# MahdiGhafoorian/NLML_HPE

Measured on AMD Instinct MI355X. Metric: faces_per_sec, higher is better.
Workload: dtype f16x2s

## Files before the change

nlml_hpe_amd/csrc/encoder_heads_f16x2_w8.hip:

```cpp
#include <hip/hip_runtime.h>

#include "../../include/nlml_hpe.h"
#include "abi_internal.h"
#include "ipd_norm.h"
#include "encoder_heads_f16x2_dev.h"
#include "layout.h"

namespace nlml {
namespace hx {

template <typename XHi, typename XLo, typename Extra>
__device__ __forceinline__ void step_w8(f32x16 (&acc)[2][2], f32x16 (&accS)[2][2], const h8 (&wcur)[2][2], const h8 (&xh)[2], h8 (&xl)[2],
                                        h8 (&wnext_hi)[2][2], const h8* __restrict__ wp_hi, h8 (&wnext_lo)[2][2], const h8* __restrict__ wp_lo,
                                        XHi xload_hi, XLo xload_lo, Extra extra) {
#pragma unroll
  for (int m = 0; m < 12; ++m) {
    const int t = m / 4, nb = (m % 4) / 2, fb = m % 2;
    if (t == 0) accS[nb][fb] = __builtin_amdgcn_mfma_f32_32x32x16_f16(wcur[nb][1], xh[fb], accS[nb][fb], 0, 0, 0);
    else if (t == 1) accS[nb][fb] = __builtin_amdgcn_mfma_f32_32x32x16_f16(wcur[nb][0], xl[fb], accS[nb][fb], 0, 0, 0);
    else acc[nb][fb] = __builtin_amdgcn_mfma_f32_32x32x16_f16(wcur[nb][0], xh[fb], acc[nb][fb], 0, 0, 0);
    __builtin_amdgcn_sched_barrier(0);
    if (m == 0) xload_hi(0);
    if (m == 1) xload_hi(1);
    if (m == 2) wnext_hi[0][0] = wp_hi[0];
    if (m == 4) wnext_lo[0][1] = wp_lo[64];
    if (m == 6) wnext_hi[1][0] = wp_hi[128];
    if (m == 8) xload_lo(0);
    if (m == 9) xload_lo(1);
    if (m == 10) wnext_lo[1][1] = wp_lo[192];
    extra(m);
    __builtin_amdgcn_sched_barrier(0);
  }
}

template <bool VEC4, bool NORM>
__device__ __forceinline__ void stage_e0_pass_w8(const Ctx& c, const Args& a, int64_t row0, int tid, int pass, int jw, int nbh,
                                                 f32x16 (&acc)[2][2], f32x16 (&accS)[2][2]) {
  constexpr int NB = 2, NFB = 2;
  constexpr int WSTEP = 4 * 2 * 64;
  const int F = a.F;
  const int nslab = (int)c.hdr.k8_e0 / XS_STEPS;

  const int srow = tid >> 3, scol = (tid & 7) * 4;
  int64_t r = row0 + srow;
  const bool live = r < a.B;
  r = live ? r : a.B - 1;
  const float* p = a.x + r * a.ldx;
  double ipd = 1.0, rcp = 1.0, ra = 0.0, rb = 0.0, rc = 0.0;
  if (NORM) {
    double x0, y0, z0;
    ipd_setup(p, ipd, rcp, x0, y0, z0);
    ipd_phase(scol % 3, x0, y0, z0, ra, rb, rc);
  }
  unsigned nzbits = 0u;

  struct Set { float v[4]; };
  auto gload = [&](int s, Set& st) {
    s = s < nslab ? s : nslab - 1;
    const int k = s * XS_COLS + scol;
    if (VEC4) {
      const int kc = k < F ? k : (NORM ? k - 12 * ((k - F + 15) / 12) : F - 4);
      const f32x4 t = *reinterpret_cast<const f32x4*>(p + kc);
#pragma unroll
      for (int e = 0; e < 4; ++e) st.v[e] = t[e];
    } else {
#pragma unroll
      for (int e = 0; e < 4; ++e) st.v[e] = p[k + e < F ? k + e : F - 1];
    }
  };
  auto lw_begin = [&](Set& st) {
#pragma unroll
    for (int e = 0; e < 4; ++e) asm volatile("" : "+v"(st.v[e]));
  };
  auto lw_norm = [&](Set& st, int q) {
    const int t = q % 3;
    const double rr = t == 0 ? ra : (t == 1 ? rb : rc);
    st.v[q] = (float)div_ipd((double)st.v[q] - rr, ipd, rcp);
  };
  auto lw_rotate = [&]() {
    const double t0 = rc; rc = rb; rb = ra; ra = t0;
  };
  typedef unsigned u2 __attribute__((ext_vector_type(2)));
  unsigned pend_hi[2], pend_lo[2];
  auto lw_split = [&](Set& st, int j, bool real_slab) {
    const unsigned m = real_slab ? 0x7fffffffu : 0u;
    nzbits |= (__float_as_uint(st.v[2 * j]) | __float_as_uint(st.v[2 * j + 1])) & m;
    split2(st.v[2 * j], st.v[2 * j + 1], pend_hi[j], pend_lo[j]);
  };
  constexpr int XW_PLANE = 64 * 64, XW_SLAB = 2 * XW_PLANE, XW_BUF = 2 * XW_SLAB, O_XW = LDS_BYTES - 2 * XW_BUF;
  static_assert(O_XW >= 16 * 512 * 16, "slabs behind the parked accumulators");
  const int wr_off = srow * 64 + ((((tid & 7) >> 1) ^ ((srow >> 2) & 3)) << 4) + 8 * (tid & 1);
  auto lw_store = [&](int slab_off, int piece) {
    char* d = c.lds + O_XW + slab_off + wr_off;
    if (piece == 0) *reinterpret_cast<u2*>(d) = u2{pend_hi[0], pend_hi[1]};
    else *reinterpret_cast<u2*>(d + XW_PLANE) = u2{pend_lo[0], pend_lo[1]};
  };
  auto lwrite = [&](int slab_off, Set& st, bool real_slab) {
    lw_begin(st);
    if (NORM) {
#pragma unroll
      for (int q = 0; q < 4; ++q) lw_norm(st, q);
      lw_rotate();
    }
#pragma unroll
    for (int j = 0; j < 2; ++j) lw_split(st, j, real_slab);
    lw_store(slab_off, 0);
    lw_store(slab_off, 1);
  };

  const int job = 4 * pass + jw;
  load_bias<NB, NFB>(acc, c.blob4 + c.hdr.b_off(ST_E0) + job * (4 * 8) + (2 * nbh) * 8, c.h);
  zero_acc<NB, NFB>(accS);
  const h8* w = c.blob8 + c.hdr.w_off(ST_E0) + (size_t)job * c.hdr.job_w16(ST_E0) + (2 * nbh * 2) * 64 + c.lane;
  auto wfrag = [&](int ks) { return w + (size_t)ks * WSTEP; };

  Set set[2];
#ifndef W8_D0_HI
#define W8_D0_HI 2
#endif
#ifndef W8_D0_LO
#define W8_D0_LO 2
#endif
  constexpr int R0 = 4, DH = W8_D0_HI, DL = W8_D0_LO;
  h8 wr[R0][NB][2];
  gload(0, set[0]);
  gload(1, set[1]);
  lwrite(0, set[0], true);
  lwrite(XW_SLAB, set[1], true);
  gload(2, set[0]);
  gload(3, set[1]);
#pragma unroll
  for (int d = 0; d < (DH > DL ? DH : DL); ++d)
#pragma unroll
    for (int nb = 0; nb < NB; ++nb)
#pragma unroll
      for (int pp = 0; pp < 2; ++pp)
        if (d < (pp ? DL : DH)) wr[d][nb][pp] = wfrag(d)[(nb * 2 + pp) * 64];
  __syncthreads();

  const int rd0 = c.f * 64 + ((c.h ^ ((c.f >> 2) & 3)) << 4);
  typedef __attribute__((address_space(3))) const char LdsC;
  LdsC* const xb0 = (LdsC*)(c.lds + O_XW + rd0);
  LdsC* const xb1 = (LdsC*)(c.lds + O_XW + (rd0 ^ 32));
  h8 xh[2][NFB], xl[NFB];
  auto xread = [&](LdsC* base, int t, int fb, int pp) {
    return *reinterpret_cast<const __attribute__((address_space(3))) h8*>(base + (t >> 1) * XW_SLAB + pp * XW_PLANE + fb * (32 * 64));
  };
  const int niter = nslab / 2;
#pragma unroll
  for (int fb = 0; fb < NFB; ++fb) {
    xh[0][fb] = xread(xb0, 0, fb, 0);
    xl[fb] = xread(xb0, 0, fb, 1);
  }
  int cur = 0, nxt = XW_BUF;
  for (int it = 0; it < niter; ++it) {
    const int s = 2 * it;
    LdsC* xc[2] = {xb0 + cur, xb1 + cur};
    LdsC* xn = xb0 + nxt;
    asm volatile("" : "+v"(xc[0]), "+v"(xc[1]), "+v"(xn));
#pragma unroll
    for (int t = 0; t < 4; ++t) {
      const int ks = 4 * it + t;
      if (t == 3) __syncthreads();
      step_w8(acc, accS, wr[t], xh[t & 1], xl, wr[(t + DH) % R0], wfrag(ks + DH), wr[(t + DL) % R0], wfrag(ks + DL),
              [&](int fb) { xh[(t + 1) & 1][fb] = t < 3 ? xread(xc[(t + 1) & 1], t + 1, fb, 0) : xread(xn, 0, fb, 0); },
              [&](int fb) { xl[fb] = t < 3 ? xread(xc[(t + 1) & 1], t + 1, fb, 1) : xread(xn, 0, fb, 1); },
              [&](int m) {
                if (t >= 2) return;
                Set& st = set[t & 1];
                const int j = m;
                const bool real = s + t + 2 < nslab;
                if (j == 0) lw_begin(st);
                if (NORM && j >= 1 && j < 5) lw_norm(st, j - 1);
                if (NORM && j == 5) lw_rotate();
                if (j == 6 || j == 7) lw_split(st, j - 6, real);
                if (j == 8) lw_store(nxt + t * XW_SLAB, 0);
                if (j == 9) lw_store(nxt + t * XW_SLAB, 1);
                if (j == 11) gload(s + t + 4, st);
              });
    }
    const int t0 = cur; cur = nxt; nxt = t0;
  }
  if (pass == 0 && a.valid) {
    const unsigned long long m = __ballot(nzbits != 0u);
    if ((tid & 7) == 0 && live) a.valid[row0 + srow] = ((m >> (c.lane & 56)) & 0xFFull) ? 1 : 0;
  }
}

#ifdef HX_STAMPS
#define W8S(i)                                                                                                          \
  do {                                                                                                                  \
    if (a.latent && c.lane == 0)                                                                                        \
      reinterpret_cast<unsigned long long*>(a.latent)[((size_t)blockIdx.x * 8 + c.wv) * 16 + (i)] = __builtin_amdgcn_s_memtime(); \
  } while (0)
#define W8S_WALL(i)                                                                                                     \
  do {                                                                                                                  \
    if (a.latent && c.lane == 0)                                                                                        \
      reinterpret_cast<unsigned long long*>(a.latent)[((size_t)blockIdx.x * 8 + c.wv) * 16 + (i)] = wall_clock64();     \
  } while (0)
#else
#define W8S(i) do { } while (0)
#define W8S_WALL(i) do { } while (0)
#endif

template <bool VEC4, bool NORM, bool TRUNK = false>
__global__ __launch_bounds__(512) void encoder_heads_f16x2_w8_kernel(Args a) {
  __shared__ __attribute__((aligned(16))) char lds[LDS_BYTES];

  const int tid = threadIdx.x;
  Ctx c;
  c.blob8 = reinterpret_cast<const h8*>(a.blob);
  c.blob4 = reinterpret_cast<const f32x4*>(a.blob);
  c.hdr = load_hdr(reinterpret_cast<const Header*>(a.blob));
  c.lds = lds;
  c.lane = tid & 63;
  c.f = c.lane & 31;
  c.h = c.lane >> 5;
  c.wv = __builtin_amdgcn_readfirstlane(tid >> 6);
  const int jw = c.wv >> 1, nbh = c.wv & 1;
  const int64_t row0 = (int64_t)blockIdx.x * TILE_FACES;

  {
    constexpr int WSTEP1 = 4 * 2 * 64;
    const h8* w1 = c.blob8 + c.hdr.w_off(ST_E1) + (size_t)jw * c.hdr.job_w16(ST_E1) + (2 * nbh * 2) * 64 + c.lane;
    const float inv0 = c.hdr.inv_scale[ST_E0];
    f32x16 acc1[2][2];
    f32x4* const park = reinterpret_cast<f32x4*>(c.lds + O_H1H) + tid;
    static_assert(16 * 512 * 16 <= 2 * P_H1H, "the parked layer-1 accumulators fit the h1 half image");
    load_bias<2, 2>(acc1, c.blob4 + c.hdr.b_off(ST_E1) + jw * (4 * 8) + (2 * nbh) * 8, c.h);
    auto park_acc1 = [&]() {
#pragma unroll
      for (int nb = 0; nb < 2; ++nb)
#pragma unroll
        for (int fb = 0; fb < 2; ++fb)
#pragma unroll
          for (int q = 0; q < 4; ++q)
            park[512 * ((nb * 2 + fb) * 4 + q)] = f32x4{acc1[nb][fb][4 * q], acc1[nb][fb][4 * q + 1], acc1[nb][fb][4 * q + 2], acc1[nb][fb][4 * q + 3]};
    };
    park_acc1();
    W8S(0);
    W8S_WALL(14);
#pragma unroll 1
    for (int pass = 0; pass < 2; ++pass) {
      {
        f32x16 acc0[2][2], acc0s[2][2];
        stage_e0_pass_w8<VEC4, NORM>(c, a, row0, tid, pass, jw, nbh, acc0, acc0s);
        add_acc<2, 2>(acc0, acc0s);
        W8S(1 + 4 * pass);
#pragma unroll
        for (int nb = 0; nb < 2; ++nb)
#pragma unroll
          for (int fb = 0; fb < 2; ++fb)
#pragma unroll
            for (int q = 0; q < 4; ++q) {
              const f32x4 t = park[512 * ((nb * 2 + fb) * 4 + q)];
              acc1[nb][fb][4 * q] = t[0]; acc1[nb][fb][4 * q + 1] = t[1]; acc1[nb][fb][4 * q + 2] = t[2]; acc1[nb][fb][4 * q + 3] = t[3];
            }
        __syncthreads();
        job_store<2, 2, ACT_RELU>(c, acc0, O_H1H, P_H1H, S_H1H, 128 * jw + 64 * nbh, 0, inv0);
      }
      __syncthreads();
      W8S(2 + 4 * pass);
      {
        f32x16 acc1s[2][2];
        zero_acc<2, 2>(acc1s);
        kloop<2, 2, 32, WSTEP1>(acc1, acc1s, w1 + (size_t)pass * 32 * WSTEP1, c.lds + O_H1H + (c.f * S_H1H + 8 * c.h) * 2, P_H1H,
                                32 * S_H1H * 2);
        add_acc<2, 2>(acc1, acc1s);
      }
      W8S(3 + 4 * pass);
      __syncthreads();
      if (pass == 0) park_acc1();
      W8S(4 + 4 * pass);
    }
    job_store<2, 2, ACT_RELU>(c, acc1, O_H2, P_H2, S_H2, 128 * jw + 64 * nbh, 0, c.hdr.inv_scale[ST_E1]);
  }
  __syncthreads();
  W8S(9);
  Ctx ct = c;
  ct.wv = c.wv & 3;
  f32x16 acc3[1][2];
  h8 wr3[ring_slots(1, 2)][1][2];
  {
    constexpr int WSTEP2 = 2 * 2 * 64;
    f32x16 acc2[1][2], acc2s[1][2];
    load_bias<1, 2>(acc2, c.blob4 + c.hdr.b_off(ST_E2) + jw * (2 * 8) + nbh * 8, c.h);
    zero_acc<1, 2>(acc2s);
    const h8* w2 = c.blob8 + c.hdr.w_off(ST_E2) + (size_t)jw * c.hdr.job_w16(ST_E2) + (nbh * 2) * 64 + c.lane;
    kloop<1, 2, 32, WSTEP2>(acc2, acc2s, w2, c.lds + O_H2 + (c.f * S_H2 + 8 * c.h) * 2, P_H2, 32 * S_H2 * 2);
    add_acc<1, 2>(acc2, acc2s);
    W8S(10);
    if constexpr (TRUNK) {
      typedef unsigned u4_ __attribute__((ext_vector_type(4)));
      u4_* const dst = reinterpret_cast<u4_*>(a.h3ws) + (size_t)blockIdx.x * (2 * 16 * 2 * 64) + c.lane;
#pragma unroll
      for (int fb = 0; fb < 2; ++fb) {
        h8 fr[2][2];
        frags_from_acc<ACT_RELU>(acc2[0][fb], c.hdr.inv_scale[ST_E2], fr);
#pragma unroll
        for (int p = 0; p < 2; ++p)
#pragma unroll
          for (int pc = 0; pc < 2; ++pc)
            dst[((fb * 16 + 4 * jw + 2 * nbh + p) * 2 + pc) * 64] = __builtin_bit_cast(u4_, fr[p][pc]);
      }
      return;
    }
    tail_pre_e3<false>(ct, acc3, wr3);
    __syncthreads();
    job_store<1, 2, ACT_RELU>(c, acc2, O_H3, P_H3, S_H3, 64 * jw + 32 * nbh, 0, c.hdr.inv_scale[ST_E2]);
  }
  __syncthreads();
  W8S(11);
  W8S_WALL(15);
  ct.helper = c.wv >= 4 ? 1 : 0;
  constexpr bool H1W8 = true;
#ifdef HX_STAMPS
  Args at = a;
  if (a.latent) at.latent = a.latent + (size_t)gridDim.x * 8 * 16 * 2;
  tail_stages<false, STRICT_INKERNEL_RESCUE_MAX, H1W8>(ct, at, row0, acc3, wr3);
#else
  tail_stages<false, STRICT_INKERNEL_RESCUE_MAX, H1W8>(ct, a, row0, acc3, wr3);
#endif
}

}

size_t tailws_workspace_bytes(int64_t B, int F) {
  if (B <= 0 || F <= 0) return 0;
  return (size_t)((B + TILE_FACES - 1) / TILE_FACES) * (2 * 16 * 2 * 1024);
}

int launch_encoder_heads_f16x2_tailws(const float* x, int64_t ldx, const float* raw, int normalize, int64_t B, int F,
                                      const void* blob, float* out, float* latent, uint8_t* valid, void* workspace,
                                      size_t ws_bytes, void* stream) {
  if (B == 0) return 0;
  if (!workspace || ws_bytes < tailws_workspace_bytes(B, F)) return fail(NLML_E_BADARG, "streamed-tail path: workspace too small");
  if (reinterpret_cast<uintptr_t>(workspace) & 15) return fail(NLML_E_BADARG, "streamed-tail path: workspace must be 16-byte aligned");
  hx::Args a;
  a.B = B; a.F = F; a.blob = blob; a.out = out; a.latent = latent; a.valid = valid; a.h3ws = workspace;
  const K2Input in = k2_input(x, ldx, raw, normalize, F);
  a.x = in.src; a.ldx = in.ld; a.norm = in.norm;
  if (!in.vec4) return fail(NLML_E_BADARG, "streamed-tail path: x must be 16-byte aligned with F and ldx multiples of 4");
  const int64_t ntiles = (B + TILE_FACES - 1) / TILE_FACES;
  const dim3 grid((unsigned)ntiles), block(512);
  hipStream_t st = reinterpret_cast<hipStream_t>(stream);
  if (a.norm) hipLaunchKernelGGL((hx::encoder_heads_f16x2_w8_kernel<true, true, true>), grid, block, 0, st, a);
  else hipLaunchKernelGGL((hx::encoder_heads_f16x2_w8_kernel<true, false, true>), grid, block, 0, st, a);
  if (int rc = hip_launch_status()) return rc;
  if (int rc = launch_tail_ws(blob, workspace, 2 * ntiles, B, out, latent, stream)) return rc;
  return launch_strict_reeval(x, ldx, raw, normalize, B, F, blob, out, latent, stream);
}

int launch_encoder_heads_f16x2_w8(const float* x, int64_t ldx, const float* raw, int normalize, int64_t B, int F,
                                  const void* blob, float* out, float* latent, uint8_t* valid, void* stream) {
  if (B == 0) return 0;
  hx::Args a;
  a.B = B; a.F = F; a.blob = blob; a.out = out; a.latent = latent; a.valid = valid;
  const K2Input in = k2_input(x, ldx, raw, normalize, F);
  a.x = in.src; a.ldx = in.ld; a.norm = in.norm;
  const dim3 grid((unsigned)((B + TILE_FACES - 1) / TILE_FACES)), block(512);
  hipStream_t st = reinterpret_cast<hipStream_t>(stream);
  k2_with_variant(in, [&](auto V, auto N) {
    hipLaunchKernelGGL((hx::encoder_heads_f16x2_w8_kernel<decltype(V)::value, decltype(N)::value>), grid, block, 0, st, a);
  });
  if (int rc = hip_launch_status()) return rc;
  return launch_strict_reeval(x, ldx, raw, normalize, B, F, blob, out, latent, stream);
}

}
```

Baseline: 80.17 million.

## Recompute lane fields per pass and defer layer-1 bias load to cut live registers

Result: no change. 80.88 million, median of 6 (+0.9%).

```diff
diff --git a/nlml_hpe_amd/csrc/encoder_heads_f16x2_w8.hip b/nlml_hpe_amd/csrc/encoder_heads_f16x2_w8.hip
--- a/nlml_hpe_amd/csrc/encoder_heads_f16x2_w8.hip
+++ b/nlml_hpe_amd/csrc/encoder_heads_f16x2_w8.hip
@@ -42,10 +42,8 @@
   const int nslab = (int)c.hdr.k8_e0 / XS_STEPS;
 
   const int srow = tid >> 3, scol = (tid & 7) * 4;
-  int64_t r = row0 + srow;
-  const bool live = r < a.B;
-  r = live ? r : a.B - 1;
-  const float* p = a.x + r * a.ldx;
+  const int nlive = (int)(a.B - row0 < TILE_FACES ? a.B - row0 : TILE_FACES);
+  const float* p = a.x + (row0 + (srow < nlive ? srow : nlive - 1)) * a.ldx;
   double ipd = 1.0, rcp = 1.0, ra = 0.0, rb = 0.0, rc = 0.0;
   if (NORM) {
     double x0, y0, z0;
@@ -116,12 +114,15 @@
 
   Set set[2];
 #ifndef W8_D0_HI
-#define W8_D0_HI 2
+#define W8_D0_HI 3
 #endif
 #ifndef W8_D0_LO
 #define W8_D0_LO 2
 #endif
   constexpr int R0 = 4, DH = W8_D0_HI, DL = W8_D0_LO;
+  static_assert((DH > DL ? DH : DL) * WSTEP <= kStages[ST_E0].jobs * kStages[ST_E0].nb * 8 + kStages[ST_E1].jobs * stage_job_w16_const(ST_E1),
+                "layer 0's weight ring stays inside the blob");
+  static_assert(DH < R0 && DL < R0 && DH >= 1 && DL >= 1, "ring depth");
   h8 wr[R0][NB][2];
   gload(0, set[0]);
   gload(1, set[1]);
@@ -183,19 +184,19 @@
   }
   if (pass == 0 && a.valid) {
     const unsigned long long m = __ballot(nzbits != 0u);
-    if ((tid & 7) == 0 && live) a.valid[row0 + srow] = ((m >> (c.lane & 56)) & 0xFFull) ? 1 : 0;
+    if ((tid & 7) == 0 && srow < nlive) a.valid[row0 + srow] = ((m >> (c.lane & 56)) & 0xFFull) ? 1 : 0;
   }
 }
 
 #ifdef HX_STAMPS
 #define W8S(i)                                                                                                          \
   do {                                                                                                                  \
-    if (a.latent && c.lane == 0)                                                                                        \
+    if (a.latent && (threadIdx.x & 63) == 0)                                                                                        \
       reinterpret_cast<unsigned long long*>(a.latent)[((size_t)blockIdx.x * 8 + c.wv) * 16 + (i)] = __builtin_amdgcn_s_memtime(); \
   } while (0)
 #define W8S_WALL(i)                                                                                                     \
   do {                                                                                                                  \
-    if (a.latent && c.lane == 0)                                                                                        \
+    if (a.latent && (threadIdx.x & 63) == 0)                                                                                        \
       reinterpret_cast<unsigned long long*>(a.latent)[((size_t)blockIdx.x * 8 + c.wv) * 16 + (i)] = wall_clock64();     \
   } while (0)
 #else
@@ -207,74 +208,85 @@
 __global__ __launch_bounds__(512) void encoder_heads_f16x2_w8_kernel(Args a) {
   __shared__ __attribute__((aligned(16))) char lds[LDS_BYTES];
 
-  const int tid = threadIdx.x;
   Ctx c;
   c.blob8 = reinterpret_cast<const h8*>(a.blob);
   c.blob4 = reinterpret_cast<const f32x4*>(a.blob);
   c.hdr = load_hdr(reinterpret_cast<const Header*>(a.blob));
   c.lds = lds;
-  c.lane = tid & 63;
-  c.f = c.lane & 31;
-  c.h = c.lane >> 5;
-  c.wv = __builtin_amdgcn_readfirstlane(tid >> 6);
+  auto lane_fields = [](Ctx& cc) {
+    unsigned z = 0;
+    asm volatile("" : "+v"(z));
+    const int t = cc.wv * 64 + (int)__builtin_amdgcn_mbcnt_hi(~0u, __builtin_amdgcn_mbcnt_lo(~0u, z));
+    cc.lane = t & 63;
+    cc.f = cc.lane & 31;
+    cc.h = cc.lane >> 5;
+    return t;
+  };
+  c.lane = c.f = c.h = 0;
+  c.wv = __builtin_amdgcn_readfirstlane((int)threadIdx.x >> 6);
   const int jw = c.wv >> 1, nbh = c.wv & 1;
   const int64_t row0 = (int64_t)blockIdx.x * TILE_FACES;
 
   {
     constexpr int WSTEP1 = 4 * 2 * 64;
-    const h8* w1 = c.blob8 + c.hdr.w_off(ST_E1) + (size_t)jw * c.hdr.job_w16(ST_E1) + (2 * nbh * 2) * 64 + c.lane;
     const float inv0 = c.hdr.inv_scale[ST_E0];
-    f32x16 acc1[2][2];
-    f32x4* const park = reinterpret_cast<f32x4*>(c.lds + O_H1H) + tid;
     static_assert(16 * 512 * 16 <= 2 * P_H1H, "the parked layer-1 accumulators fit the h1 half image");
-    load_bias<2, 2>(acc1, c.blob4 + c.hdr.b_off(ST_E1) + jw * (4 * 8) + (2 * nbh) * 8, c.h);
-    auto park_acc1 = [&]() {
-#pragma unroll
-      for (int nb = 0; nb < 2; ++nb)
-#pragma unroll
-        for (int fb = 0; fb < 2; ++fb)
-#pragma unroll
-          for (int q = 0; q < 4; ++q)
-            park[512 * ((nb * 2 + fb) * 4 + q)] = f32x4{acc1[nb][fb][4 * q], acc1[nb][fb][4 * q + 1], acc1[nb][fb][4 * q + 2], acc1[nb][fb][4 * q + 3]};
-    };
-    park_acc1();
     W8S(0);
     W8S_WALL(14);
 #pragma unroll 1
     for (int pass = 0; pass < 2; ++pass) {
+      Ctx cp = c;
+      const int tp = lane_fields(cp);
+      f32x16 acc1[2][2];
+      f32x4* const park = reinterpret_cast<f32x4*>(cp.lds + O_H1H) + tp;
       {
         f32x16 acc0[2][2], acc0s[2][2];
-        stage_e0_pass_w8<VEC4, NORM>(c, a, row0, tid, pass, jw, nbh, acc0, acc0s);
+        stage_e0_pass_w8<VEC4, NORM>(cp, a, row0, tp, pass, jw, nbh, acc0, acc0s);
         add_acc<2, 2>(acc0, acc0s);
         W8S(1 + 4 * pass);
-#pragma unroll
-        for (int nb = 0; nb < 2; ++nb)
-#pragma unroll
-          for (int fb = 0; fb < 2; ++fb)
-#pragma unroll
-            for (int q = 0; q < 4; ++q) {
-              const f32x4 t = park[512 * ((nb * 2 + fb) * 4 + q)];
-              acc1[nb][fb][4 * q] = t[0]; acc1[nb][fb][4 * q + 1] = t[1]; acc1[nb][fb][4 * q + 2] = t[2]; acc1[nb][fb][4 * q + 3] = t[3];
-            }
+        if (pass == 0) {
+          load_bias<2, 2>(acc1, cp.blob4 + cp.hdr.b_off(ST_E1) + jw * (4 * 8) + (2 * nbh) * 8, cp.h);
+        } else {
+#pragma unroll
+          for (int nb = 0; nb < 2; ++nb)
+#pragma unroll
+            for (int fb = 0; fb < 2; ++fb)
+#pragma unroll
+              for (int q = 0; q < 4; ++q) {
+                const f32x4 t = park[512 * ((nb * 2 + fb) * 4 + q)];
+                acc1[nb][fb][4 * q] = t[0]; acc1[nb][fb][4 * q + 1] = t[1]; acc1[nb][fb][4 * q + 2] = t[2]; acc1[nb][fb][4 * q + 3] = t[3];
+              }
+        }
         __syncthreads();
-        job_store<2, 2, ACT_RELU>(c, acc0, O_H1H, P_H1H, S_H1H, 128 * jw + 64 * nbh, 0, inv0);
+        job_store<2, 2, ACT_RELU>(cp, acc0, O_H1H, P_H1H, S_H1H, 128 * jw + 64 * nbh, 0, inv0);
       }
       __syncthreads();
       W8S(2 + 4 * pass);
       {
+        const h8* w1 = cp.blob8 + cp.hdr.w_off(ST_E1) + (size_t)jw * cp.hdr.job_w16(ST_E1) + (2 * nbh * 2) * 64 + cp.lane;
         f32x16 acc1s[2][2];
         zero_acc<2, 2>(acc1s);
-        kloop<2, 2, 32, WSTEP1>(acc1, acc1s, w1 + (size_t)pass * 32 * WSTEP1, c.lds + O_H1H + (c.f * S_H1H + 8 * c.h) * 2, P_H1H,
+        kloop<2, 2, 32, WSTEP1>(acc1, acc1s, w1 + (size_t)pass * 32 * WSTEP1, cp.lds + O_H1H + (cp.f * S_H1H + 8 * cp.h) * 2, P_H1H,
                                 32 * S_H1H * 2);
         add_acc<2, 2>(acc1, acc1s);
       }
       W8S(3 + 4 * pass);
       __syncthreads();
-      if (pass == 0) park_acc1();
+      if (pass == 0) {
+#pragma unroll
+        for (int nb = 0; nb < 2; ++nb)
+#pragma unroll
+          for (int fb = 0; fb < 2; ++fb)
+#pragma unroll
+            for (int q = 0; q < 4; ++q)
+              park[512 * ((nb * 2 + fb) * 4 + q)] = f32x4{acc1[nb][fb][4 * q], acc1[nb][fb][4 * q + 1], acc1[nb][fb][4 * q + 2], acc1[nb][fb][4 * q + 3]};
+      } else {
+        job_store<2, 2, ACT_RELU>(cp, acc1, O_H2, P_H2, S_H2, 128 * jw + 64 * nbh, 0, cp.hdr.inv_scale[ST_E1]);
+      }
       W8S(4 + 4 * pass);
     }
-    job_store<2, 2, ACT_RELU>(c, acc1, O_H2, P_H2, S_H2, 128 * jw + 64 * nbh, 0, c.hdr.inv_scale[ST_E1]);
-  }
+  }
+  lane_fields(c);
   __syncthreads();
   W8S(9);
   Ctx ct = c;
```
